# serviceberry3/weiner_slamit_v2

Measured on AMD Instinct MI355X. Metric: frames/sec ORB extract+match @640x480x8lvl, higher is better.
Workload: dtype u8; 1 GPU; BASELINE configs[1]: 640x480 8-level ORB extract (1000 features, FAST 20/7) + brute-force 256-bit Hamming best/second match vs the stream's previous frame; 256 independent streams per GPU per step; distinct_frame_pairs_per_gpu=16, parallelism=streams sharded over 1 GPU(s), no data-path collective

## Files before the change

### weiner_slamit_v2_amd/csrc/hamming.hip

```cpp
#include <hip/hip_runtime.h>
#include <stdint.h>
#include <stdlib.h>
#include <string.h>

#include <algorithm>

#include "../../include/slamit.h"
#include "slamit_internal.h"

#define HM_TILE 256
#ifndef HM_SLICES
#define HM_SLICES 8
#endif
#define HM_QPB (256 / HM_SLICES)

__device__ __forceinline__ unsigned bcnt_acc(unsigned x, unsigned acc) {
    unsigned r;
    asm("v_bcnt_u32_b32 %0, %1, %2" : "=v"(r) : "v"(x), "v"(acc));
    return r;
}
__device__ __forceinline__ unsigned umed3(unsigned a, unsigned b, unsigned c) {
    unsigned r;
    asm("v_med3_u32 %0, %1, %2, %3" : "=v"(r) : "v"(a), "v"(b), "v"(c));
    return r;
}

__global__ __launch_bounds__(256) void hamming_best2_kernel(
    const uint8_t* __restrict__ q, const int* __restrict__ nq_arr, int nq_fixed, size_t q_stride,
    const uint8_t* __restrict__ t, const int* __restrict__ nt_arr, int nt_fixed, size_t t_stride,
    int* __restrict__ best_idx, int* __restrict__ best, int* __restrict__ second, size_t out_stride) {
    __shared__ uint4 tile[HM_TILE * 2];
    const int pair = blockIdx.y;
    const int nq = nq_arr ? nq_arr[pair] : nq_fixed;
    const int nt = nt_arr ? nt_arr[pair] : nt_fixed;
    const int tid = threadIdx.x;
    const int qi = blockIdx.x * HM_QPB + tid / HM_SLICES;
    const int slice = tid % HM_SLICES;
    if (blockIdx.x * HM_QPB >= nq) return;
    const uint4* Q = reinterpret_cast<const uint4*>(q + (size_t)pair * q_stride);
    const uint4* T = reinterpret_cast<const uint4*>(t + (size_t)pair * t_stride);
    uint4 a0 = make_uint4(0, 0, 0, 0), a1 = a0;
    const bool live = qi < nq;
    if (live) { a0 = Q[2 * (size_t)qi]; a1 = Q[2 * (size_t)qi + 1]; }
    unsigned kb = 0xFFFFFFFFu, ks = 0xFFFFFFFFu;
    const uint4 zero = make_uint4(0, 0, 0, 0);
    uint4 p0 = zero, p1 = zero;
    if (nt > 0) {
        const int last = 2 * min(nt, HM_TILE) - 1;
        p0 = T[min(tid, last)]; p1 = T[min(tid + 256, last)];
    }
    for (int base = 0; base < nt; base += HM_TILE) {
        const int rows = min(HM_TILE, nt - base);
        __syncthreads();
        tile[tid] = p0; tile[tid + 256] = p1;
        __syncthreads();
        if (base + HM_TILE < nt) {
            const int last = 2 * min(HM_TILE, nt - base - HM_TILE) - 1;
            const uint4* Tn = T + 2 * (size_t)(base + HM_TILE);
            p0 = Tn[min(tid, last)]; p1 = Tn[min(tid + 256, last)];
        }
#define HM_DIST(T0, T1) bcnt_acc(a1.w ^ T1.w, bcnt_acc(a1.z ^ T1.z, bcnt_acc(a1.y ^ T1.y, bcnt_acc(a1.x ^ T1.x, \
                        bcnt_acc(a0.w ^ T0.w, bcnt_acc(a0.z ^ T0.z, bcnt_acc(a0.y ^ T0.y, bcnt_acc(a0.x ^ T0.x, 0u))))))))
#define HM_TAKE(D, J) do { const unsigned k = ((D) << 16) | (unsigned)(base + (J)); \
            ks = umed3(kb, ks, k);    \
            kb = min(kb, k); } while (0)
        int j = slice;
        for (; j + 3 * HM_SLICES < rows; j += 4 * HM_SLICES) {
            const uint4 t00 = tile[2 * j], t01 = tile[2 * j + 1], t10 = tile[2 * (j + HM_SLICES)], t11 = tile[2 * (j + HM_SLICES) + 1];
            const uint4 t20 = tile[2 * (j + 2 * HM_SLICES)], t21 = tile[2 * (j + 2 * HM_SLICES) + 1];
            const uint4 t30 = tile[2 * (j + 3 * HM_SLICES)], t31 = tile[2 * (j + 3 * HM_SLICES) + 1];
            const unsigned d0 = HM_DIST(t00, t01), d1 = HM_DIST(t10, t11), d2 = HM_DIST(t20, t21), d3 = HM_DIST(t30, t31);
            HM_TAKE(d0, j); HM_TAKE(d1, j + HM_SLICES); HM_TAKE(d2, j + 2 * HM_SLICES); HM_TAKE(d3, j + 3 * HM_SLICES);
        }
        for (; j < rows; j += HM_SLICES) { const uint4 t0 = tile[2 * j], t1 = tile[2 * j + 1]; const unsigned d = HM_DIST(t0, t1); HM_TAKE(d, j); }
#undef HM_DIST
#undef HM_TAKE
    }
#pragma unroll
    for (int m = 1; m < HM_SLICES; m <<= 1) {
        const unsigned ob = (unsigned)__shfl_xor((int)kb, m, 64), os = (unsigned)__shfl_xor((int)ks, m, 64);
        ks = min(min(ks, os), max(kb, ob));
        kb = min(kb, ob);
    }
    const int b = kb == 0xFFFFFFFFu ? 256 : (int)(kb >> 16), bi = kb == 0xFFFFFFFFu ? -1 : (int)(kb & 0xFFFFu);
    const int s = ks == 0xFFFFFFFFu ? 256 : (int)(ks >> 16);
    if (live && slice == 0) {
        size_t o = (size_t)pair * out_stride + qi;
        best_idx[o] = bi; best[o] = b; second[o] = s;
    }
}

typedef int hm_v4i __attribute__((ext_vector_type(4)));
typedef int hm_v16i __attribute__((ext_vector_type(16)));
#define HMM_MAX_TRAIN 8192
#define HMM_NONE 0x40000000
#define HMM_EMPTY 0x7F000000

__device__ __forceinline__ hm_v4i hm_unpack_q(const uint4 w, const int s) {
    const unsigned hi = 0x80808080u, mid = 0x40404040u;
    hm_v4i r;
    r.x = (int)__builtin_amdgcn_bitop3_b32(w.x << (7 - s), hi, mid, 0xEA);
    r.y = (int)__builtin_amdgcn_bitop3_b32(w.y << (7 - s), hi, mid, 0xEA);
    r.z = (int)__builtin_amdgcn_bitop3_b32(w.z << (7 - s), hi, mid, 0xEA);
    r.w = (int)__builtin_amdgcn_bitop3_b32(w.w << (7 - s), hi, mid, 0xEA);
    return r;
}
__device__ __forceinline__ hm_v4i hm_unpack_t(const uint4 w, const int s) {
    const unsigned hi = 0x80808080u, mid = 0x40404040u;
    hm_v4i r;
    r.x = (int)__builtin_amdgcn_bitop3_b32(w.x << (7 - s), hi, mid, 0xAE);
    r.y = (int)__builtin_amdgcn_bitop3_b32(w.y << (7 - s), hi, mid, 0xAE);
    r.z = (int)__builtin_amdgcn_bitop3_b32(w.z << (7 - s), hi, mid, 0xAE);
    r.w = (int)__builtin_amdgcn_bitop3_b32(w.w << (7 - s), hi, mid, 0xAE);
    return r;
}
__device__ __forceinline__ int imed3_after(int a, int b, int c, int after) {
    int r;
    asm("v_med3_i32 %0, %1, %2, %3" : "=v"(r) : "v"(a), "v"(b), "v"(c), "v"(after));
    return r;
}

#define HMM_WAVES 4
#define HMM_NT 4

__device__ __forceinline__ void hm_merge2(int& kb, int& ks, int ob, int os) {
    ks = min(min(ks, os), max(kb, ob));
    kb = min(kb, ob);
}

__global__ __launch_bounds__(64 * HMM_WAVES) __attribute__((amdgpu_waves_per_eu(2, 2))) void hamming_best2_mfma_kernel(
    const uint8_t* __restrict__ q, const int* __restrict__ nq_arr, int nq_fixed, size_t q_stride,
    const uint8_t* __restrict__ t, const int* __restrict__ nt_arr, int nt_fixed, size_t t_stride,
    int* __restrict__ best_idx, int* __restrict__ best, int* __restrict__ second, size_t out_stride) {
    __shared__ int s_keys[HMM_WAVES - 1][64][2 * HMM_NT];
    const int pair = blockIdx.y;
    const int nq = __builtin_amdgcn_readfirstlane(nq_arr ? nq_arr[pair] : nq_fixed);
    const int nt = __builtin_amdgcn_readfirstlane(min(nt_arr ? nt_arr[pair] : nt_fixed, HMM_MAX_TRAIN));
    const int qbase = blockIdx.x * 32 * HMM_NT;
    if (qbase >= nq) return;
    const int wv = __builtin_amdgcn_readfirstlane(threadIdx.x >> 6);
    const int lane = threadIdx.x & 63;
    const int col = lane & 31, h = lane >> 5;
    const uint4* Q = reinterpret_cast<const uint4*>(q + (size_t)pair * q_stride);
    const uint4* T = reinterpret_cast<const uint4*>(t + (size_t)pair * t_stride);
    hm_v4i bq[HMM_NT][8];
#pragma unroll
    for (int u = 0; u < HMM_NT; ++u) {
        const uint4 w = Q[2 * (size_t)min(qbase + 32 * u + col, nq - 1) + h];
#pragma unroll
        for (int s = 0; s < 8; ++s) bq[u][s] = hm_unpack_q(w, s);
    }
    hm_v16i cinit;
#pragma unroll
    for (int r = 0; r < 16; ++r) cinit[r] = 4 * h + (r & 3) + 8 * (r >> 2);
    int kb[HMM_NT], ks[HMM_NT];
#pragma unroll
    for (int u = 0; u < HMM_NT; ++u) kb[u] = ks[u] = HMM_EMPTY;
    const int ntiles = (nt + 31) >> 5;
    uint4 wt = make_uint4(0u, 0u, 0u, 0u);
    if (wv < ntiles) wt = T[2 * (size_t)min(wv * 32 + col, nt - 1) + h];
    int tile = wv;
    for (; tile < ntiles; tile += HMM_WAVES) {
        const uint4 w = wt;
        if (tile + HMM_WAVES < ntiles) wt = T[2 * (size_t)min((tile + HMM_WAVES) * 32 + col, nt - 1) + h];
        hm_v16i c[HMM_NT];
        {
            const hm_v4i a = hm_unpack_t(w, 0);
            hm_v16i cm = cinit;
            if (tile * 32 + 32 > nt) {
#pragma unroll
                for (int r = 0; r < 16; ++r) cm[r] = tile * 32 + cinit[r] < nt ? cinit[r] : HMM_NONE;
            }
#pragma unroll
            for (int u = 0; u < HMM_NT; ++u) c[u] = __builtin_amdgcn_mfma_i32_32x32x32_i8(a, bq[u][0], cm, 0, 0, 0);
        }
#pragma unroll
        for (int s = 1; s < 8; ++s) {
            const hm_v4i a = hm_unpack_t(w, s);
#pragma unroll
            for (int u = 0; u < HMM_NT; ++u) c[u] = __builtin_amdgcn_mfma_i32_32x32x32_i8(a, bq[u][s], c[u], 0, 0, 0);
        }
        if (tile != wv) {
#pragma unroll
            for (int u = 0; u < HMM_NT; ++u) { kb[u] -= 32 * HMM_WAVES; ks[u] -= 32 * HMM_WAVES; }
        }
#pragma unroll
        for (int u = 0; u < HMM_NT; ++u) {
#pragma unroll
            for (int r = 0; r < 16; ++r) {
                const int n = min(kb[u], c[u][r]);
                ks[u] = imed3_after(kb[u], ks[u], c[u][r], n);
                kb[u] = n;
            }
        }
    }
    if (tile != wv) {
        const int base = (tile - HMM_WAVES) * 32;
#pragma unroll
        for (int u = 0; u < HMM_NT; ++u) { kb[u] += base; ks[u] += base; }
    }
#pragma unroll
    for (int u = 0; u < HMM_NT; ++u) hm_merge2(kb[u], ks[u], __shfl_xor(kb[u], 32, 64), __shfl_xor(ks[u], 32, 64));
    if (wv > 0) {
#pragma unroll
        for (int u = 0; u < HMM_NT; ++u) { s_keys[wv - 1][lane][2 * u] = kb[u]; s_keys[wv - 1][lane][2 * u + 1] = ks[u]; }
    }
    __syncthreads();
    if (wv != 0 || h != 0) return;
#pragma unroll
    for (int o = 0; o < HMM_WAVES - 1; ++o) {
#pragma unroll
        for (int u = 0; u < HMM_NT; ++u) hm_merge2(kb[u], ks[u], s_keys[o][lane][2 * u], s_keys[o][lane][2 * u + 1]);
    }
#pragma unroll
    for (int u = 0; u < HMM_NT; ++u) {
        const int qi = qbase + 32 * u + col;
        if (qi >= nq) continue;
        const bool hb = kb[u] < 0x20000000, hs = ks[u] < 0x20000000;
        const size_t o = (size_t)pair * out_stride + qi;
        best_idx[o] = hb ? ((kb[u] + (1 << 20)) & 8191) : -1;
        best[o] = hb ? ((kb[u] + (1 << 20)) >> 13) : 256;
        second[o] = hs ? ((ks[u] + (1 << 20)) >> 13) : 256;
    }
}

__global__ __launch_bounds__(256) void hamming_matrix_kernel(const uint8_t* __restrict__ q, int nq,
                                                             const uint8_t* __restrict__ t, int nt,
                                                             uint16_t* __restrict__ out) {
    __shared__ uint4 tile[64 * 2];
    const int tid = threadIdx.x;
    const int j0 = blockIdx.x * 64, i0 = blockIdx.y * 64;
    const uint4* Q = reinterpret_cast<const uint4*>(q);
    const uint4* T = reinterpret_cast<const uint4*>(t);
    const int rows = min(64, nt - j0);
    for (int i = tid; i < rows * 2; i += 256) tile[i] = T[2 * (size_t)j0 + i];
    __syncthreads();
    const int j = tid & 63;
    for (int ii = tid >> 6; ii < 64; ii += 4) {
        int i = i0 + ii;
        if (i >= nq || j >= rows) continue;
        uint4 a0 = Q[2 * (size_t)i], a1 = Q[2 * (size_t)i + 1];
        uint4 t0 = tile[2 * j], t1 = tile[2 * j + 1];
        int d = __popc(a0.x ^ t0.x) + __popc(a0.y ^ t0.y) + __popc(a0.z ^ t0.z) + __popc(a0.w ^ t0.w) +
                __popc(a1.x ^ t1.x) + __popc(a1.y ^ t1.y) + __popc(a1.z ^ t1.z) + __popc(a1.w ^ t1.w);
        out[(size_t)i * nt + j0 + j] = (uint16_t)d;
    }
}

__global__ __launch_bounds__(64) void distinctive_kernel(const uint8_t* __restrict__ desc, const int* __restrict__ offsets,
                                                         int* __restrict__ best_idx, int* __restrict__ best_median) {
    __shared__ uint4 rowsd[SLAMIT_DISTINCTIVE_MAX * 2];
    __shared__ unsigned short D[SLAMIT_DISTINCTIVE_MAX * SLAMIT_DISTINCTIVE_MAX];
    const int p = blockIdx.x, lane = threadIdx.x;
    const int o = offsets[p], n = offsets[p + 1] - o;
    if (n <= 0) { if (lane == 0) { best_idx[p] = -1; best_median[p] = 0; } return; }
    const uint4* G = reinterpret_cast<const uint4*>(desc + (size_t)o * 32);
    for (int i = lane; i < 2 * n; i += 64) rowsd[i] = G[i];
    __builtin_amdgcn_fence(__ATOMIC_ACQ_REL, "wavefront");
    __builtin_amdgcn_wave_barrier();
    for (int i = lane; i < n; i += 64) {
        const uint4 a0 = rowsd[2 * i], a1 = rowsd[2 * i + 1];
        for (int j = 0; j < n; ++j) {
            const uint4 t0 = rowsd[2 * j], t1 = rowsd[2 * j + 1];
            const int d = __popc(a0.x ^ t0.x) + __popc(a0.y ^ t0.y) + __popc(a0.z ^ t0.z) + __popc(a0.w ^ t0.w) +
                          __popc(a1.x ^ t1.x) + __popc(a1.y ^ t1.y) + __popc(a1.z ^ t1.z) + __popc(a1.w ^ t1.w);
            D[i * n + j] = (unsigned short)d;
        }
    }
    const int k = (int)(0.5 * (n - 1));
    unsigned bestkey = 0xFFFFFFFFu;
    for (int i = lane; i < n; i += 64) {
        int lo = 0, hi = 256;
        while (lo < hi) {
            const int mid = (lo + hi) >> 1;
            int c = 0;
            for (int j = 0; j < n; ++j) c += D[i * n + j] <= mid;
            if (c >= k + 1) hi = mid; else lo = mid + 1;
        }
        bestkey = min(bestkey, ((unsigned)lo << 16) | (unsigned)i);
    }
#pragma unroll
    for (int d = 32; d >= 1; d >>= 1) bestkey = min(bestkey, (unsigned)__shfl_xor((int)bestkey, d, 64));
    if (lane == 0) { best_idx[p] = (int)(bestkey & 0xFFFF); best_median[p] = (int)(bestkey >> 16); }
}

static bool hm_use_mfma(int max_train) { return max_train <= HMM_MAX_TRAIN; }

extern "C" {

int slamit_distinctive_batch(const uint8_t* desc, const int32_t* offsets, int npoints, int32_t* best_idx,
                             int32_t* best_median) {
    if (npoints < 0 || (npoints && (!offsets || !best_idx || !best_median))) return slamit_fail(SLAMIT_ERR_ARG, "slamit_distinctive_batch: bad argument");
    if (npoints == 0) return SLAMIT_OK;
    for (int p = 0; p < npoints; ++p) {
        const int n = offsets[p + 1] - offsets[p];
        if (n < 0 || offsets[0] < 0) return slamit_fail(SLAMIT_ERR_ARG, "slamit_distinctive_batch: offsets must be non-decreasing");
        if (n > SLAMIT_DISTINCTIVE_MAX) return slamit_fail(SLAMIT_ERR_CAPACITY, "slamit_distinctive_batch: more than SLAMIT_DISTINCTIVE_MAX rows for one point");
    }
    const int total = offsets[npoints];
    if (total && !desc) return slamit_fail(SLAMIT_ERR_ARG, "slamit_distinctive_batch: null descriptors");
    const int cur_dev = slamit_default_device();
    SLAMIT_USE_DEVICE(cur_dev);
    StageLayout L;
    const StageSpan<uint8_t> d = L.take<uint8_t>(32 * (size_t)total);
    const StageSpan<int> off = L.take<int>((size_t)npoints + 1);
    L.end_inputs();
    const StageSpan<int> idx = L.take<int>(npoints), med = L.take<int>(npoints, alignof(int));
    L.end_outputs();
    static thread_local SlamitScratch S;
    HIP_TRY_AT("slamit_distinctive_batch", slamit_stage_reserve(S, cur_dev, L));
    if (total) memcpy(d.at(S.host), desc, d.bytes());
    memcpy(off.at(S.host), offsets, off.bytes());
    HIP_TRY_AT("slamit_distinctive_batch", slamit_stage_upload(S, L));
    hipLaunchKernelGGL(distinctive_kernel, dim3(npoints), dim3(64), 0, S.st, d.at(S.dev), off.at(S.dev), idx.at(S.dev), med.at(S.dev));
    HIP_TRY_AT("slamit_distinctive_batch", slamit_stage_download_and_wait(S, L));
    memcpy(best_idx, idx.at(S.host), idx.bytes());
    memcpy(best_median, med.at(S.host), med.bytes());
    return SLAMIT_OK;
}

int slamit_hamming_best2_batch_dev(const uint8_t* d_q, const int32_t* d_nq, size_t q_stride, const uint8_t* d_t,
                                   const int32_t* d_nt, size_t t_stride, int npairs, int max_n,
                                   int32_t* d_best_idx, int32_t* d_best, int32_t* d_second, size_t out_stride,
                                   int device, void* stream) {
    if (npairs < 0 || max_n < 0 || !d_q || !d_t || !d_nq || !d_nt || !d_best_idx || !d_best || !d_second)
        return slamit_fail(SLAMIT_ERR_ARG, "slamit_hamming_best2_batch_dev: bad argument");
    if ((q_stride & 15) || (t_stride & 15) || ((uintptr_t)d_q & 15) || ((uintptr_t)d_t & 15))
        return slamit_fail(SLAMIT_ERR_ARG, "slamit_hamming_best2_batch_dev: descriptors must be 16-byte aligned");
    if (npairs == 0 || max_n == 0) return SLAMIT_OK;
    if (max_n > SLAMIT_HAMMING_MAX_TRAIN) return slamit_fail(SLAMIT_ERR_CAPACITY, "slamit_hamming_best2_batch_dev: more than SLAMIT_HAMMING_MAX_TRAIN descriptors per set");
    SLAMIT_USE_DEVICE(device);
    if (hm_use_mfma(max_n)) {
        hipLaunchKernelGGL(hamming_best2_mfma_kernel, dim3((max_n + 32 * HMM_NT - 1) / (32 * HMM_NT), npairs), dim3(64 * HMM_WAVES), 0, (hipStream_t)stream, d_q, d_nq, 0, q_stride,
                           d_t, d_nt, 0, t_stride, d_best_idx, d_best, d_second, out_stride);
    } else {
        dim3 grid((max_n + HM_QPB - 1) / HM_QPB, npairs);
        hipLaunchKernelGGL(hamming_best2_kernel, grid, dim3(256), 0, (hipStream_t)stream, d_q, d_nq, 0, q_stride, d_t, d_nt,
                           0, t_stride, d_best_idx, d_best, d_second, out_stride);
    }
    HIP_TRY(hipGetLastError());
    return SLAMIT_OK;
}

int slamit_hamming_best2(const uint8_t* q, int nq, const uint8_t* t, int nt, int32_t* best_idx, int32_t* best,
                         int32_t* second) {
    if (nq < 0 || nt < 0 || (nq && (!q || !best_idx || !best || !second)) || (nt && !t))
        return slamit_fail(SLAMIT_ERR_ARG, "slamit_hamming_best2: bad argument");
    if (nq == 0) return SLAMIT_OK;
    if (nt > SLAMIT_HAMMING_MAX_TRAIN) return slamit_fail(SLAMIT_ERR_CAPACITY, "slamit_hamming_best2: more than SLAMIT_HAMMING_MAX_TRAIN train descriptors");
    const int cur_dev = slamit_default_device();
    SLAMIT_USE_DEVICE(cur_dev);
    StageLayout L;
    const StageSpan<uint8_t> dq = L.take<uint8_t>(32 * (size_t)nq), dt = L.take<uint8_t>(32 * (size_t)std::max(nt, 1));
    L.end_inputs();
    const StageSpan<int> idx = L.take<int>(nq), b1 = L.take<int>(nq, alignof(int)), b2 = L.take<int>(nq, alignof(int));
    L.end_outputs();
    static thread_local SlamitScratch S;
    HIP_TRY_AT("slamit_hamming_best2", slamit_stage_reserve(S, cur_dev, L));
    memcpy(dq.at(S.host), q, dq.bytes());
    if (nt) memcpy(dt.at(S.host), t, 32 * (size_t)nt);
    HIP_TRY_AT("slamit_hamming_best2", slamit_stage_upload(S, L));
    if (hm_use_mfma(nt))
        hipLaunchKernelGGL(hamming_best2_mfma_kernel, dim3((nq + 32 * HMM_NT - 1) / (32 * HMM_NT), 1), dim3(64 * HMM_WAVES), 0, S.st, dq.at(S.dev), (const int*)nullptr, nq,
                           (size_t)0, dt.at(S.dev), (const int*)nullptr, nt, (size_t)0, idx.at(S.dev), b1.at(S.dev), b2.at(S.dev), (size_t)0);
    else
        hipLaunchKernelGGL(hamming_best2_kernel, dim3((nq + HM_QPB - 1) / HM_QPB, 1), dim3(256), 0, S.st, dq.at(S.dev), (const int*)nullptr, nq,
                           (size_t)0, dt.at(S.dev), (const int*)nullptr, nt, (size_t)0, idx.at(S.dev), b1.at(S.dev), b2.at(S.dev), (size_t)0);
    HIP_TRY_AT("slamit_hamming_best2", slamit_stage_download_and_wait(S, L));
    memcpy(best_idx, idx.at(S.host), idx.bytes()); memcpy(best, b1.at(S.host), b1.bytes()); memcpy(second, b2.at(S.host), b2.bytes());
    return SLAMIT_OK;
}

int slamit_hamming_matrix(const uint8_t* q, int nq, const uint8_t* t, int nt, uint16_t* out) {
    if (nq < 0 || nt < 0 || ((nq && nt) && (!q || !t || !out))) return slamit_fail(SLAMIT_ERR_ARG, "slamit_hamming_matrix: bad argument");
    if (nq == 0 || nt == 0) return SLAMIT_OK;
    const int cur_dev = slamit_default_device();
    SLAMIT_USE_DEVICE(cur_dev);
    StageLayout L;
    const StageSpan<uint8_t> dq = L.take<uint8_t>(32 * (size_t)nq), dt = L.take<uint8_t>(32 * (size_t)nt);
    L.end_inputs();
    const StageSpan<uint16_t> d = L.take<uint16_t>((size_t)nq * nt);
    L.end_outputs();
    static thread_local SlamitScratch S;
    HIP_TRY_AT("slamit_hamming_matrix", slamit_stage_reserve(S, cur_dev, L));
    memcpy(dq.at(S.host), q, dq.bytes());
    memcpy(dt.at(S.host), t, dt.bytes());
    HIP_TRY_AT("slamit_hamming_matrix", slamit_stage_upload(S, L));
    hipLaunchKernelGGL(hamming_matrix_kernel, dim3((nt + 63) / 64, (nq + 63) / 64), dim3(256), 0, S.st, dq.at(S.dev), nq, dt.at(S.dev), nt, d.at(S.dev));
    HIP_TRY_AT("slamit_hamming_matrix", slamit_stage_download_and_wait(S, L));
    memcpy(out, d.at(S.host), d.bytes());
    return SLAMIT_OK;
}

}
```

Measured before the change: 309,200 frames/s.

## Switch Hamming matching MFMA from int8 to scaled FP4 32x32x64

Bits are now unpacked into 4-bit FP4 values (±1 encoding), and the distance/index key is accumulated with the scaled f8f6f4 MFMA into float accumulators. This halves the number of MFMA steps per tile (4 instead of 8) and the unpack work. The best/second tracking now uses float med3 and integer min on the float bit patterns, with an exponent scale of 133 and a bias of 2^21 to keep integer keys exact in float. Risks are float precision of the packed index/distance key and the correctness of the FP4 encoding and scale choice.

```diff
diff --git a/weiner_slamit_v2_amd/csrc/hamming.hip b/weiner_slamit_v2_amd/csrc/hamming.hip
--- a/weiner_slamit_v2_amd/csrc/hamming.hip
+++ b/weiner_slamit_v2_amd/csrc/hamming.hip
@@ -90,49 +90,57 @@
     }
 }
 
-typedef int hm_v4i __attribute__((ext_vector_type(4)));
-typedef int hm_v16i __attribute__((ext_vector_type(16)));
+typedef int hm_v8i __attribute__((ext_vector_type(8)));
+typedef float hm_v16f __attribute__((ext_vector_type(16)));
 #define HMM_MAX_TRAIN 8192
-#define HMM_NONE 0x40000000
-#define HMM_EMPTY 0x7F000000
-
-__device__ __forceinline__ hm_v4i hm_unpack_q(const uint4 w, const int s) {
-    const unsigned hi = 0x80808080u, mid = 0x40404040u;
-    hm_v4i r;
-    r.x = (int)__builtin_amdgcn_bitop3_b32(w.x << (7 - s), hi, mid, 0xEA);
-    r.y = (int)__builtin_amdgcn_bitop3_b32(w.y << (7 - s), hi, mid, 0xEA);
-    r.z = (int)__builtin_amdgcn_bitop3_b32(w.z << (7 - s), hi, mid, 0xEA);
-    r.w = (int)__builtin_amdgcn_bitop3_b32(w.w << (7 - s), hi, mid, 0xEA);
+#define HMM_NONE 0x1p30f
+#define HMM_EMPTY 0x1p30f
+#define HMM_BIAS 0x1p21f
+#define HMM_LIVE 0x1p29f
+#define HMM_FP4 4
+#define HMM_SCALE 133
+
+__device__ __forceinline__ hm_v8i hm_unpack_q(const uint4 w, const int s) {
+    const unsigned sign = 0x88888888u, one = 0x22222222u;
+    hm_v8i r = {};
+    r[0] = (int)__builtin_amdgcn_bitop3_b32(w.x << (3 - s), sign, one, 0xEA);
+    r[1] = (int)__builtin_amdgcn_bitop3_b32(w.y << (3 - s), sign, one, 0xEA);
+    r[2] = (int)__builtin_amdgcn_bitop3_b32(w.z << (3 - s), sign, one, 0xEA);
+    r[3] = (int)__builtin_amdgcn_bitop3_b32(w.w << (3 - s), sign, one, 0xEA);
     return r;
 }
-__device__ __forceinline__ hm_v4i hm_unpack_t(const uint4 w, const int s) {
-    const unsigned hi = 0x80808080u, mid = 0x40404040u;
-    hm_v4i r;
-    r.x = (int)__builtin_amdgcn_bitop3_b32(w.x << (7 - s), hi, mid, 0xAE);
-    r.y = (int)__builtin_amdgcn_bitop3_b32(w.y << (7 - s), hi, mid, 0xAE);
-    r.z = (int)__builtin_amdgcn_bitop3_b32(w.z << (7 - s), hi, mid, 0xAE);
-    r.w = (int)__builtin_amdgcn_bitop3_b32(w.w << (7 - s), hi, mid, 0xAE);
+__device__ __forceinline__ hm_v8i hm_unpack_t(const uint4 w, const int s) {
+    const unsigned sign = 0x88888888u, one = 0x22222222u;
+    hm_v8i r = {};
+    r[0] = (int)__builtin_amdgcn_bitop3_b32(w.x << (3 - s), sign, one, 0xAE);
+    r[1] = (int)__builtin_amdgcn_bitop3_b32(w.y << (3 - s), sign, one, 0xAE);
+    r[2] = (int)__builtin_amdgcn_bitop3_b32(w.z << (3 - s), sign, one, 0xAE);
+    r[3] = (int)__builtin_amdgcn_bitop3_b32(w.w << (3 - s), sign, one, 0xAE);
     return r;
 }
-__device__ __forceinline__ int imed3_after(int a, int b, int c, int after) {
-    int r;
-    asm("v_med3_i32 %0, %1, %2, %3" : "=v"(r) : "v"(a), "v"(b), "v"(c), "v"(after));
-    return r;
+__device__ __forceinline__ hm_v16f hm_mfma(const hm_v8i a, const hm_v8i b, const hm_v16f c) {
+    return __builtin_amdgcn_mfma_scale_f32_32x32x64_f8f6f4(a, b, c, HMM_FP4, HMM_FP4, 0, HMM_SCALE, 0, HMM_SCALE);
 }
 
 #define HMM_WAVES 4
+#ifndef HMM_NT
 #define HMM_NT 4
-
-__device__ __forceinline__ void hm_merge2(int& kb, int& ks, int ob, int os) {
-    ks = min(min(ks, os), max(kb, ob));
-    kb = min(kb, ob);
+#endif
+#define HMM_NG 4
+
+__device__ __forceinline__ float hm_min(float a, float b) { return __int_as_float(min(__float_as_int(a), __float_as_int(b))); }
+__device__ __forceinline__ float hm_max(float a, float b) { return __int_as_float(max(__float_as_int(a), __float_as_int(b))); }
+
+__device__ __forceinline__ void hm_merge2(float& kb, float& ks, float ob, float os) {
+    ks = hm_min(hm_min(ks, os), hm_max(kb, ob));
+    kb = hm_min(kb, ob);
 }
 
 __global__ __launch_bounds__(64 * HMM_WAVES) __attribute__((amdgpu_waves_per_eu(2, 2))) void hamming_best2_mfma_kernel(
     const uint8_t* __restrict__ q, const int* __restrict__ nq_arr, int nq_fixed, size_t q_stride,
     const uint8_t* __restrict__ t, const int* __restrict__ nt_arr, int nt_fixed, size_t t_stride,
     int* __restrict__ best_idx, int* __restrict__ best, int* __restrict__ second, size_t out_stride) {
-    __shared__ int s_keys[HMM_WAVES - 1][64][2 * HMM_NT];
+    __shared__ float s_keys[HMM_WAVES - 1][64][2 * HMM_NT];
     const int pair = blockIdx.y;
     const int nq = __builtin_amdgcn_readfirstlane(nq_arr ? nq_arr[pair] : nq_fixed);
     const int nt = __builtin_amdgcn_readfirstlane(min(nt_arr ? nt_arr[pair] : nt_fixed, HMM_MAX_TRAIN));
@@ -143,17 +151,17 @@
     const int col = lane & 31, h = lane >> 5;
     const uint4* Q = reinterpret_cast<const uint4*>(q + (size_t)pair * q_stride);
     const uint4* T = reinterpret_cast<const uint4*>(t + (size_t)pair * t_stride);
-    hm_v4i bq[HMM_NT][8];
+    hm_v8i bq[HMM_NT][4];
 #pragma unroll
     for (int u = 0; u < HMM_NT; ++u) {
         const uint4 w = Q[2 * (size_t)min(qbase + 32 * u + col, nq - 1) + h];
 #pragma unroll
-        for (int s = 0; s < 8; ++s) bq[u][s] = hm_unpack_q(w, s);
-    }
-    hm_v16i cinit;
-#pragma unroll
-    for (int r = 0; r < 16; ++r) cinit[r] = 4 * h + (r & 3) + 8 * (r >> 2);
-    int kb[HMM_NT], ks[HMM_NT];
+        for (int s = 0; s < 4; ++s) bq[u][s] = hm_unpack_q(w, s);
+    }
+    hm_v16f cinit;
+#pragma unroll
+    for (int r = 0; r < 16; ++r) cinit[r] = HMM_BIAS + (float)(4 * h + (r & 3) + 8 * (r >> 2));
+    float kb[HMM_NT], ks[HMM_NT];
 #pragma unroll
     for (int u = 0; u < HMM_NT; ++u) kb[u] = ks[u] = HMM_EMPTY;
     const int ntiles = (nt + 31) >> 5;
@@ -163,39 +171,40 @@
     for (; tile < ntiles; tile += HMM_WAVES) {
         const uint4 w = wt;
         if (tile + HMM_WAVES < ntiles) wt = T[2 * (size_t)min((tile + HMM_WAVES) * 32 + col, nt - 1) + h];
-        hm_v16i c[HMM_NT];
-        {
-            const hm_v4i a = hm_unpack_t(w, 0);
-            hm_v16i cm = cinit;
-            if (tile * 32 + 32 > nt) {
-#pragma unroll
-                for (int r = 0; r < 16; ++r) cm[r] = tile * 32 + cinit[r] < nt ? cinit[r] : HMM_NONE;
+        hm_v8i a[4];
+#pragma unroll
+        for (int s = 0; s < 4; ++s) a[s] = hm_unpack_t(w, s);
+        if (tile * 32 + 32 > nt) {
+#pragma unroll
+            for (int r = 0; r < 16; ++r) cinit[r] = tile * 32 + 4 * h + (r & 3) + 8 * (r >> 2) < nt ? cinit[r] : HMM_NONE;
+        }
+        if (tile != wv) {
+#pragma unroll
+            for (int u = 0; u < HMM_NT; ++u) { kb[u] -= 32 * HMM_WAVES; ks[u] -= 32 * HMM_WAVES; }
+        }
+#pragma unroll
+        for (int g = 0; g < HMM_NT; g += HMM_NG) {
+            hm_v16f c[HMM_NG];
+#pragma unroll
+            for (int u = 0; u < HMM_NG; ++u) c[u] = hm_mfma(a[0], bq[g + u][0], cinit);
+#pragma unroll
+            for (int s = 1; s < 4; ++s) {
+#pragma unroll
+                for (int u = 0; u < HMM_NG; ++u) c[u] = hm_mfma(a[s], bq[g + u][s], c[u]);
             }
 #pragma unroll
-            for (int u = 0; u < HMM_NT; ++u) c[u] = __builtin_amdgcn_mfma_i32_32x32x32_i8(a, bq[u][0], cm, 0, 0, 0);
-        }
-#pragma unroll
-        for (int s = 1; s < 8; ++s) {
-            const hm_v4i a = hm_unpack_t(w, s);
-#pragma unroll
-            for (int u = 0; u < HMM_NT; ++u) c[u] = __builtin_amdgcn_mfma_i32_32x32x32_i8(a, bq[u][s], c[u], 0, 0, 0);
-        }
-        if (tile != wv) {
-#pragma unroll
-            for (int u = 0; u < HMM_NT; ++u) { kb[u] -= 32 * HMM_WAVES; ks[u] -= 32 * HMM_WAVES; }
-        }
-#pragma unroll
-        for (int u = 0; u < HMM_NT; ++u) {
-#pragma unroll
-            for (int r = 0; r < 16; ++r) {
-                const int n = min(kb[u], c[u][r]);
-                ks[u] = imed3_after(kb[u], ks[u], c[u][r], n);
-                kb[u] = n;
+            for (int u = 0; u < HMM_NG; ++u) {
+#pragma unroll
+                for (int r = 0; r < 16; ++r) {
+                    const float k = c[u][r];
+                    ks[g + u] = __builtin_amdgcn_fmed3f(kb[g + u], ks[g + u], k);
+                    kb[g + u] = hm_min(kb[g + u], k);
+                }
             }
         }
     }
     if (tile != wv) {
-        const int base = (tile - HMM_WAVES) * 32;
+        const float base = (float)((tile - HMM_WAVES) * 32);
 #pragma unroll
         for (int u = 0; u < HMM_NT; ++u) { kb[u] += base; ks[u] += base; }
     }
@@ -216,11 +225,12 @@
     for (int u = 0; u < HMM_NT; ++u) {
         const int qi = qbase + 32 * u + col;
         if (qi >= nq) continue;
-        const bool hb = kb[u] < 0x20000000, hs = ks[u] < 0x20000000;
+        const bool hb = kb[u] < HMM_LIVE, hs = ks[u] < HMM_LIVE;
+        const int ib = (int)kb[u] - (1 << 20), is = (int)ks[u] - (1 << 20);
         const size_t o = (size_t)pair * out_stride + qi;
-        best_idx[o] = hb ? ((kb[u] + (1 << 20)) & 8191) : -1;
-        best[o] = hb ? ((kb[u] + (1 << 20)) >> 13) : 256;
-        second[o] = hs ? ((ks[u] + (1 << 20)) >> 13) : 256;
+        best_idx[o] = hb ? (ib & 8191) : -1;
+        best[o] = hb ? (ib >> 13) : 256;
+        second[o] = hs ? (is >> 13) : 256;
     }
 }
 
```

Result: faster. 315,100 frames/s, median of 6 (+1.9%).
